# neggles/neurosis

Hardware: AMD Instinct MI355X
Metric: train images/sec (node) SDXL 1024^2 (higher is better)
Workload: dtype bf16

## Files before the change

include/neurosis_hip.h:

```cpp
#ifndef NEUROSIS_HIP_H
#define NEUROSIS_HIP_H

#ifdef __cplusplus
extern "C" {
#endif

const char* nk_last_error(void);
int nk_abi_version(void);

int nk_linear_fwd(const void* x, const void* w, const float* bias, const void* residual, void* y,
                  int M, int N, int K, long ldx, long ldw, long ldr, long ldy, float alpha, void* stream);
int nk_linear_dgrad(const void* dy, const void* w, const void* dx_add, void* dx, int M, int N, int K,
                    long lddy, long ldw, long ldadd, long lddx, void* stream);
long nk_linear_fwd_geglu_ok(int M, int I, int K);
int nk_linear_fwd_geglu(const void* x, const void* w, const float* bias, void* u, void* h, int M, int I, int K, long ldx, long ldw, long ldu,
                        long ldh, void* stream);
int nk_linear_dgrad_geglu(const void* dy, const void* w, const void* u, void* du, int M, int N, int I, long lddy, long ldw, long ldu,
                          long lddu, void* stream);
int nk_linear_fwd_geglu_s(const void* x, const void* w, const float* bias, void* s, void* h, int M, int I, int K, long ldx, long ldw, long lds,
                          long ldh, void* stream);
int nk_linear_dgrad_geglu_s(const void* dy, const void* w, const void* s, void* du, int M, int N, int I, long lddy, long ldw, long lds,
                            long lddu, void* stream);
int nk_linear_wgrad(const void* dy, const void* x, float* dw, int M, int N, int K, long lddy, long ldx,
                    long lddw, int accumulate, void* stream);
// ... 65 lines not shown
int nk_groupnorm_sums(const void* x, float* sums, float* ws, int N, int HW, int C, int G, void* stream);
long nk_groupnorm_sums_ws_floats(int N, int nparts, int G);
int nk_groupnorm_sums_from_parts(const float* part, float* sums, float* ws, int N, int nparts, int G, void* stream);
int nk_groupnorm_apply(const void* x, const float* sums, const float* gamma, const float* beta, void* y, float* mean, float* rstd,
                       int N, int HW, int C, int G, float eps, int silu, void* stream);
int nk_groupnorm_bwd(const void* dy, const void* x, const float* gamma, const float* beta, const float* mean,
                     const float* rstd, const void* dx_add, void* dx, float* dgamma, float* dbeta, float* ws,
                     int N, int HW, int C, int G, int silu, int accumulate, void* stream);
int nk_groupnorm_mod_fwd(const void* x, const float* gamma, const float* beta, const void* mod, void* y, float* mean, float* rstd,
                         float* ws, int N, int HW, int C, int G, float eps, int silu, void* stream);
int nk_groupnorm_mod_apply(const void* x, const float* sums, const float* gamma, const float* beta, const void* mod, void* y, float* mean,
                           float* rstd, int N, int HW, int C, int G, float eps, int silu, void* stream);
int nk_groupnorm_mod_bwd(const void* dy, const void* x, const float* gamma, const float* beta, const void* mod, const float* mean,
                         const float* rstd, const void* dx_add, void* dx, float* dgamma, float* dbeta, void* dmod, float* ws,
                         int N, int HW, int C, int G, int silu, int accumulate, void* stream);

int nk_layernorm_fwd(const void* x, const float* gamma, const float* beta, void* y, float* mean, float* rstd,
                     int M, int C, float eps, void* stream);
long nk_layernorm_ws_floats(int M, int C);
int nk_layernorm_bwd(const void* dy, const void* x, const float* gamma, const float* mean, const float* rstd,
                     const void* dx_add, void* dx, float* dgamma, float* dbeta, float* ws, int M, int C, int accumulate, void* stream);
#define NK_COLPART_MAX 32
typedef struct NkColpartBatch {
  const float* part[NK_COLPART_MAX];
  float* dgamma[NK_COLPART_MAX];
  float* dbeta[NK_COLPART_MAX];
  int nrows[NK_COLPART_MAX];
  int C[NK_COLPART_MAX];
  int accumulate[NK_COLPART_MAX];
  int n;
// ... 142 lines not shown
```

neurosis_amd/csrc/norm.hip:

```cpp
#include "../../include/neurosis_hip.h"
#include "nk_common.h"

#define GN_THREADS 256
#define GN_MAXC 4096

__global__ __launch_bounds__(GN_THREADS) void gn_stats_kernel(const bf16_t* __restrict__ x, float* __restrict__ stats,
                                                              int HW, int C, int G, int rows_per) {
  __shared__ float ps[GN_THREADS * 8], pss[GN_THREADS * 8];
  const int n = blockIdx.y;
  const int cpr = (C >> 3) / gridDim.z;
  const int ch0 = blockIdx.z * cpr;
  const int rows_par = GN_THREADS / cpr;
  const int tid = threadIdx.x;
  const int cpg = C / G;
  const int row_lo = blockIdx.x * rows_per;
  const int row_hi = min(HW, row_lo + rows_per);
  float s[8], ss[8];
#pragma unroll
  for (int e = 0; e < 8; ++e) { s[e] = 0.f; ss[e] = 0.f; }
  const int chunk = tid % cpr, rsub = tid / cpr;
  if (rsub < rows_par) {
    const bf16_t* base = x + ((long)n * HW) * C + (ch0 + chunk) * 8;
    int r = row_lo + rsub;
    for (; r + 3 * rows_par < row_hi; r += 4 * rows_par) {
// ... 21 lines not shown
    }
  }
  __syncthreads();
  float* part = stats + (((long)n * gridDim.x + blockIdx.x) * gridDim.z + blockIdx.z) * 2 * G;
  for (int i = tid; i < 2 * G; i += GN_THREADS) {
    const int g = i >> 1;
    const float* src = (i & 1) ? pss : ps;
    const int c_lo = max(g * cpg, ch0 * 8), c_hi = min((g + 1) * cpg, (ch0 + cpr) * 8);
    float a = 0.f;
    for (int c = c_lo; c < c_hi; ++c)
      for (int r = 0; r < rows_par; ++r) a += src[r * cpr * 8 + (c - ch0 * 8)];
    part[i] = a;
  }
}

__global__ __launch_bounds__(1024) void gn_reduce_partials_kernel(const float* __restrict__ part, float* __restrict__ out,
                                                                 int nparts, int G2) {
  __shared__ float sm[8][128];
  const int n = blockIdx.x;
  const int tx = threadIdx.x & 127, ty = threadIdx.x >> 7;
  float a = 0.f;
  if (tx < G2)
    for (int p = ty; p < nparts; p += 8) a += part[((long)n * nparts + p) * G2 + tx];
  sm[ty][tx] = a;
  __syncthreads();
  if (ty == 0 && tx < G2) {
#pragma unroll
    for (int j = 1; j < 8; ++j) a += sm[j][tx];
    out[(long)n * G2 + tx] = a;
  }
}

__device__ __forceinline__ void gn_modulate(const bf16_t* __restrict__ mod, int n, int c, int C, float& ga, float& be) {
  const float s1 = 1.0f + bf2f(mod[(long)n * 2 * C + c]);
  const float t = bf2f(mod[(long)n * 2 * C + C + c]);
  ga = ga * s1;
  be = be * s1 + t;
}

template <bool MOD>
__global__ __launch_bounds__(GN_THREADS) void gn_apply_kernel(const bf16_t* __restrict__ x, const float* __restrict__ stats,
                                                              const float* __restrict__ gamma, const float* __restrict__ beta,
                                                              const bf16_t* __restrict__ mod,
                                                              bf16_t* __restrict__ y, float* __restrict__ mean_out,
                                                              float* __restrict__ rstd_out, int HW, int C, int G,
                                                              float eps, int silu, int rows_per) {
  extern __shared__ __attribute__((aligned(16))) char smem_raw[];
  float* sc = (float*)smem_raw;
  float* sh = sc + C;
  const int n = blockIdx.y;
  const int tid = threadIdx.x;
  const int cpg = C / G;
  const float inv_cnt = 1.0f / ((float)HW * (float)cpg);
  for (int c = tid; c < C; c += GN_THREADS) {
    int g = c / cpg;
    float m = stats[(long)n * 2 * G + 2 * g] * inv_cnt;
    float var = fmaxf(stats[(long)n * 2 * G + 2 * g + 1] * inv_cnt - m * m, 0.f);
    float rs = rsqrtf(var + eps);
    float ga = gamma[c], be = beta[c];
    if constexpr (MOD) gn_modulate(mod, n, c, C, ga, be);
    float a = rs * ga;
    sc[c] = a;
    sh[c] = be - m * a;
    if (blockIdx.x == 0 && (c % cpg) == 0) { mean_out[n * G + g] = m; rstd_out[n * G + g] = rs; }
  }
  __syncthreads();
  const int cpr = C >> 3;
  const int row_lo = blockIdx.x * rows_per;
  const int row_hi = min(HW, row_lo + rows_per);
  const unsigned total = (unsigned)(row_hi - row_lo) * (unsigned)cpr;
  const bf16_t* xb = x + ((long)n * HW + row_lo) * C;
  bf16_t* yb = y + ((long)n * HW + row_lo) * C;
// ... 180 lines not shown
  if (ty == 0 && c < C) {
#pragma unroll
    for (int j = 1; j < 16; ++j) { a += sa[j][tx]; b += sb[j][tx]; }
    dmod[(long)n * 2 * C + c] = f2bf(gamma[c] * b + beta[c] * a);
    dmod[(long)n * 2 * C + C + c] = f2bf(a);
  }
}

template <bool MOD>
__global__ __launch_bounds__(GN_THREADS) void gn_bwd_apply_kernel(const bf16_t* __restrict__ dy, const bf16_t* __restrict__ x,
                                                                  const float* __restrict__ gamma, const float* __restrict__ beta,
                                                                  const bf16_t* __restrict__ mod,
                                                                  const float* __restrict__ mean, const float* __restrict__ rstd,
                                                                  const float* __restrict__ gsum, const bf16_t* __restrict__ dx_add,
                                                                  bf16_t* __restrict__ dx, int HW, int C, int G, int silu,
                                                                  int rows_per) {
  extern __shared__ __attribute__((aligned(16))) char smem_raw[];
  float* p_a = (float*)smem_raw;
  float* p_b = p_a + C;
  float* p_c = p_b + C;
  float* p_d = p_c + C;
  const int n = blockIdx.y;
  const int tid = threadIdx.x;
  const int cpg = C / G;
  const float inv_cnt = 1.0f / ((float)HW * (float)cpg);
  for (int c = tid; c < C; c += GN_THREADS) {
    const int g = c / cpg;
    const float mu = mean[n * G + g], rs = rstd[n * G + g];
    const float s1 = gsum[(long)n * 2 * G + 2 * g] * inv_cnt, s2 = gsum[(long)n * 2 * G + 2 * g + 1] * inv_cnt;
    float ga = gamma[c], be = beta[c];
    if constexpr (MOD) gn_modulate(mod, n, c, C, ga, be);
    const float a = rs * ga;
    p_a[c] = a;
    p_b[c] = be - mu * a;
    p_c[c] = -rs * rs * s2;
    p_d[c] = -rs * s1 + mu * rs * rs * s2;
  }
  __syncthreads();
  const int cpr = C >> 3;
  const int row_lo = blockIdx.x * rows_per;
  const int row_hi = min(HW, row_lo + rows_per);
  const unsigned total = (unsigned)(row_hi - row_lo) * (unsigned)cpr;
  const long off0 = ((long)n * HW + row_lo) * C;
  auto one = [&](unsigned i, const uint4_t& rx, const uint4_t& rd, const uint4_t& ra) {
// ... 36 lines not shown

static int gn_nz(int C) {
  int cpr = C >> 3, nz = (cpr + GN_THREADS - 1) / GN_THREADS;
  while (cpr % nz) ++nz;
  return nz;
}

static int gn_rows_per(int N, int HW, int* nsplit) {
  int want = (1024 + N - 1) / N;
  int rows_per = (HW + want - 1) / want;
  if (rows_per < 32) rows_per = 32;
  *nsplit = (HW + rows_per - 1) / rows_per;
  return rows_per;
}

extern "C" long nk_groupnorm_ws_floats(int N, int HW, int C, int G) {
  int nsplit;
  gn_rows_per(N, HW, &nsplit);
  long parts = (long)N * nsplit * gn_nz(C) * 2 * G;
  long chan = (long)N * nsplit * 2 * C;
  return parts + chan + (long)N * 2 * G + 64;
}

extern "C" int nk_groupnorm_fwd(const void* x, const float* gamma, const float* beta, void* y, float* mean,
                                float* rstd, float* ws, int N, int HW, int C, int G, float eps, int silu,
                                void* stream_) {
  hipStream_t stream = (hipStream_t)stream_;
  NK_CHECK_ARG(N > 0 && HW > 0 && C > 0 && G > 0 && G <= 64);
  NK_CHECK_ARG((C & 7) == 0 && C % G == 0 && C <= GN_MAXC);
  NK_CHECK_ARG(x && gamma && beta && y && mean && rstd && ws);
  int nsplit;
  int rows_per = gn_rows_per(N, HW, &nsplit);
  const int nz = gn_nz(C);
  float* part = ws;
  float* stats = ws + (long)N * nsplit * nz * 2 * G;
  hipLaunchKernelGGL(gn_stats_kernel, dim3(nsplit, N, nz), dim3(GN_THREADS), 0, stream, (const bf16_t*)x, part, HW, C,
                     G, rows_per);
  if (int e = nk_check_launch("gn_stats_kernel")) return e;
  hipLaunchKernelGGL(gn_reduce_partials_kernel, dim3(N), dim3(1024), 0, stream, part, stats, nsplit * nz, 2 * G);
  if (int e = nk_check_launch("gn_reduce_partials_kernel")) return e;
  hipLaunchKernelGGL(gn_apply_kernel<false>, dim3(nsplit, N), dim3(GN_THREADS), 2 * C * sizeof(float), stream,
                     (const bf16_t*)x, stats, gamma, beta, (const bf16_t*)nullptr, (bf16_t*)y, mean, rstd, HW, C, G, eps, silu, rows_per);
  return nk_check_launch("gn_apply_kernel");
}

__global__ __launch_bounds__(256) void gn_reduce_partials_l1_kernel(const float* __restrict__ part, float* __restrict__ out, int nparts, int G2, int nchunks) {
  __shared__ float sm[4][64];
  const int n = blockIdx.y, chunk = blockIdx.x;
  const int tx = threadIdx.x & 63, ty = threadIdx.x >> 6;
  float a = 0.f;
  if (tx < G2)
    for (int p = chunk + ty * nchunks; p < nparts; p += 4 * nchunks) a += part[((long)n * nparts + p) * G2 + tx];
  sm[ty][tx] = a;
  __syncthreads();
  if (ty == 0 && tx < G2) out[((long)n * nchunks + chunk) * G2 + tx] = (a + sm[1][tx]) + (sm[2][tx] + sm[3][tx]);
}

extern "C" long nk_groupnorm_sums_ws_floats(int N, int nparts, int G) {
// ... 26 lines not shown
  hipLaunchKernelGGL(gn_stats_kernel, dim3(nsplit, N, nz), dim3(GN_THREADS), 0, stream, (const bf16_t*)x, ws, HW, C, G, rows_per);
  if (int e = nk_check_launch("gn_stats_kernel")) return e;
  hipLaunchKernelGGL(gn_reduce_partials_kernel, dim3(N), dim3(1024), 0, stream, ws, sums, nsplit * nz, 2 * G);
  return nk_check_launch("gn_reduce_partials_kernel");
}

extern "C" int nk_groupnorm_apply(const void* x, const float* sums, const float* gamma, const float* beta, void* y, float* mean,
                                  float* rstd, int N, int HW, int C, int G, float eps, int silu, void* stream_) {
  hipStream_t stream = (hipStream_t)stream_;
  NK_CHECK_ARG(N > 0 && HW > 0 && C > 0 && G > 0 && G <= 64);
  NK_CHECK_ARG((C & 7) == 0 && C % G == 0 && C <= GN_MAXC);
  NK_CHECK_ARG(x && sums && gamma && beta && y && mean && rstd);
  int nsplit;
  int rows_per = gn_rows_per(N, HW, &nsplit);
  hipLaunchKernelGGL(gn_apply_kernel<false>, dim3(nsplit, N), dim3(GN_THREADS), 2 * C * sizeof(float), stream, (const bf16_t*)x, sums, gamma, beta,
                     (const bf16_t*)nullptr, (bf16_t*)y, mean, rstd, HW, C, G, eps, silu, rows_per);
  return nk_check_launch("gn_apply_kernel");
}

extern "C" int nk_groupnorm_bwd(const void* dy, const void* x, const float* gamma, const float* beta,
                                const float* mean, const float* rstd, const void* dx_add, void* dx, float* dgamma,
                                float* dbeta, float* ws, int N, int HW, int C, int G, int silu, int accumulate, void* stream_) {
  hipStream_t stream = (hipStream_t)stream_;
  NK_CHECK_ARG(N > 0 && HW > 0 && C > 0 && G > 0 && G <= 64);
  NK_CHECK_ARG((C & 7) == 0 && C % G == 0 && C <= GN_MAXC);
  NK_CHECK_ARG(dy && x && gamma && beta && mean && rstd && dx && dgamma && dbeta && ws);
  int nsplit;
  int rows_per = gn_rows_per(N, HW, &nsplit);
  const int nz = gn_nz(C);
  float* part = ws;
  float* gsum = part + (long)N * nsplit * nz * 2 * G;
  float* chan = gsum + (long)N * 2 * G;
  hipLaunchKernelGGL(gn_bwd_stats_kernel<false>, dim3(nsplit, N, nz), dim3(GN_THREADS), 2 * C * sizeof(float), stream,
                     (const bf16_t*)dy, (const bf16_t*)x, gamma, beta, (const bf16_t*)nullptr, mean, rstd, part, chan, HW, C, G, silu, rows_per);
  if (int e = nk_check_launch("gn_bwd_stats_kernel")) return e;
  hipLaunchKernelGGL(gn_reduce_partials_kernel, dim3(N), dim3(1024), 0, stream, part, gsum, nsplit * nz, 2 * G);
  if (int e = nk_check_launch("gn_reduce_partials_kernel")) return e;
  hipLaunchKernelGGL(colpart_reduce_kernel, dim3((C + 63) / 64), dim3(1024), 0, stream, chan, dgamma, dbeta, N * nsplit, C, accumulate);
  if (int e = nk_check_launch("colpart_reduce_kernel")) return e;
  hipLaunchKernelGGL(gn_bwd_apply_kernel<false>, dim3(nsplit, N), dim3(GN_THREADS), 4 * C * sizeof(float), stream,
                     (const bf16_t*)dy, (const bf16_t*)x, gamma, beta, (const bf16_t*)nullptr, mean, rstd, gsum, (const bf16_t*)dx_add,
                     (bf16_t*)dx, HW, C, G, silu, rows_per);
  return nk_check_launch("gn_bwd_apply_kernel");
}

static int gn_mod_apply_launch(const void* x, const float* sums, const float* gamma, const float* beta, const void* mod, void* y, float* mean,
                               float* rstd, int N, int HW, int C, int G, float eps, int silu, hipStream_t stream) {
  int nsplit;
  int rows_per = gn_rows_per(N, HW, &nsplit);
  hipLaunchKernelGGL(gn_apply_kernel<true>, dim3(nsplit, N), dim3(GN_THREADS), 2 * C * sizeof(float), stream, (const bf16_t*)x, sums, gamma, beta,
                     (const bf16_t*)mod, (bf16_t*)y, mean, rstd, HW, C, G, eps, silu, rows_per);
  return nk_check_launch("gn_apply_kernel<mod>");
}

extern "C" int nk_groupnorm_mod_fwd(const void* x, const float* gamma, const float* beta, const void* mod, void* y, float* mean, float* rstd,
                                    float* ws, int N, int HW, int C, int G, float eps, int silu, void* stream_) {
  hipStream_t stream = (hipStream_t)stream_;
  NK_CHECK_ARG(N > 0 && HW > 0 && C > 0 && G > 0 && G <= 64);
  NK_CHECK_ARG((C & 7) == 0 && C % G == 0 && C <= GN_MAXC);
  NK_CHECK_ARG(x && gamma && beta && mod && y && mean && rstd && ws);
  int nsplit;
  gn_rows_per(N, HW, &nsplit);
  float* stats = ws + (long)N * nsplit * gn_nz(C) * 2 * G;
  if (int e = nk_groupnorm_sums(x, stats, ws, N, HW, C, G, stream_)) return e;
  return gn_mod_apply_launch(x, stats, gamma, beta, mod, y, mean, rstd, N, HW, C, G, eps, silu, stream);
}

extern "C" int nk_groupnorm_mod_apply(const void* x, const float* sums, const float* gamma, const float* beta, const void* mod, void* y,
                                      float* mean, float* rstd, int N, int HW, int C, int G, float eps, int silu, void* stream_) {
  NK_CHECK_ARG(N > 0 && HW > 0 && C > 0 && G > 0 && G <= 64);
  NK_CHECK_ARG((C & 7) == 0 && C % G == 0 && C <= GN_MAXC);
  NK_CHECK_ARG(x && sums && gamma && beta && mod && y && mean && rstd);
  return gn_mod_apply_launch(x, sums, gamma, beta, mod, y, mean, rstd, N, HW, C, G, eps, silu, (hipStream_t)stream_);
}

extern "C" int nk_groupnorm_mod_bwd(const void* dy, const void* x, const float* gamma, const float* beta, const void* mod, const float* mean,
                                    const float* rstd, const void* dx_add, void* dx, float* dgamma, float* dbeta, void* dmod, float* ws,
                                    int N, int HW, int C, int G, int silu, int accumulate, void* stream_) {
  hipStream_t stream = (hipStream_t)stream_;
  NK_CHECK_ARG(N > 0 && HW > 0 && C > 0 && G > 0 && G <= 64);
  NK_CHECK_ARG((C & 7) == 0 && C % G == 0 && C <= GN_MAXC);
  NK_CHECK_ARG(dy && x && gamma && beta && mod && mean && rstd && dx && dgamma && dbeta && dmod && ws);
  int nsplit;
  int rows_per = gn_rows_per(N, HW, &nsplit);
  const int nz = gn_nz(C);
  float* part = ws;
  float* gsum = part + (long)N * nsplit * nz * 2 * G;
  float* chan = gsum + (long)N * 2 * G;
  hipLaunchKernelGGL(gn_bwd_stats_kernel<true>, dim3(nsplit, N, nz), dim3(GN_THREADS), 2 * C * sizeof(float), stream,
                     (const bf16_t*)dy, (const bf16_t*)x, gamma, beta, (const bf16_t*)mod, mean, rstd, part, chan, HW, C, G, silu, rows_per);
  if (int e = nk_check_launch("gn_bwd_stats_kernel<mod>")) return e;
  hipLaunchKernelGGL(gn_reduce_partials_kernel, dim3(N), dim3(1024), 0, stream, part, gsum, nsplit * nz, 2 * G);
  if (int e = nk_check_launch("gn_reduce_partials_kernel")) return e;
  hipLaunchKernelGGL(colpart_reduce_mod_kernel, dim3((C + 63) / 64), dim3(1024), 0, stream, chan, (const bf16_t*)mod, dgamma, dbeta, N * nsplit,
                     nsplit, C, accumulate);
  if (int e = nk_check_launch("colpart_reduce_mod_kernel")) return e;
  hipLaunchKernelGGL(gn_dmod_kernel, dim3((C + 63) / 64, N), dim3(1024), 0, stream, chan, gamma, beta, (bf16_t*)dmod, nsplit, C);
  if (int e = nk_check_launch("gn_dmod_kernel")) return e;
  hipLaunchKernelGGL(gn_bwd_apply_kernel<true>, dim3(nsplit, N), dim3(GN_THREADS), 4 * C * sizeof(float), stream,
                     (const bf16_t*)dy, (const bf16_t*)x, gamma, beta, (const bf16_t*)mod, mean, rstd, gsum, (const bf16_t*)dx_add,
                     (bf16_t*)dx, HW, C, G, silu, rows_per);
  return nk_check_launch("gn_bwd_apply_kernel<mod>");
}

#define LN_MAXCH 4

template <int NCH>
__global__ __launch_bounds__(256) void ln_fwd_kernel(const bf16_t* __restrict__ x, const float* __restrict__ gamma,
                                                     const float* __restrict__ beta, bf16_t* __restrict__ y,
                                                     float* __restrict__ mean, float* __restrict__ rstd, int M, int C,
                                                     float eps) {
  const int lane = threadIdx.x & 63;
  const int wave = (blockIdx.x * blockDim.x + threadIdx.x) >> 6;
  const int nwaves = (gridDim.x * blockDim.x) >> 6;
  const int cpr = C >> 3;
  const float invC = 1.0f / (float)C;
// ... 398 lines not shown
```

neurosis_amd/lib.py:

```python
from __future__ import annotations

import ctypes as C
import os
from pathlib import Path

import torch

CSRC = Path(__file__).resolve().parent / "csrc"
LIB_PATH = CSRC / "libneurosis_hip.so"

vp, i32, i64, f32 = C.c_void_p, C.c_int, C.c_long, C.c_float


class NkConvDesc(C.Structure):
    _fields_ = [(n, i32) for n in ("N", "H", "W", "Cin", "Cout", "KH", "KW", "stride", "pad_t", "pad_l", "Ho", "Wo", "upsample")]


class NkAttnDesc(C.Structure):
    _fields_ = (
        [(n, i32) for n in ("B", "H", "Lq", "Lk", "D")]
        + [(n, i64) for n in ("sq", "sk", "sv", "so", "bq", "bk", "bv", "bo", "sdq", "sdk", "sdv", "sdo", "bdq", "bdk", "bdv", "bdo")]
        + [("scale", f32), ("causal", i32)]
    )

# ... 28 lines not shown
    "nk_conv2d_dgrad_flipped": [cdp, vp, vp, vp, vp],
    "nk_conv2d_wgrad": [cdp, vp, vp, vp, i32, vp],
    "nk_attention_fwd": [adp, vp, vp, vp, vp, vp, vp],
    "nk_attention_bwd": [adp, vp, vp, vp, vp, vp, vp, vp, vp, vp, vp, vp],
    "nk_attention_bwd_causal": [adp, vp, vp, vp, vp, vp, vp, vp, vp, vp, vp],
    "nk_softmax_rows": [vp, i64, i32, vp],
    "nk_softmax_rows_bwd": [vp, vp, i64, i32, f32, vp],
    "nk_groupnorm_fwd": [vp, vp, vp, vp, vp, vp, vp, i32, i32, i32, i32, f32, i32, vp],
    "nk_groupnorm_sums": [vp, vp, vp, i32, i32, i32, i32, vp],
    "nk_groupnorm_sums_from_parts": [vp, vp, vp, i32, i32, i32, vp],
    "nk_groupnorm_apply": [vp, vp, vp, vp, vp, vp, vp, i32, i32, i32, i32, f32, i32, vp],
    "nk_groupnorm_bwd": [vp, vp, vp, vp, vp, vp, vp, vp, vp, vp, vp, i32, i32, i32, i32, i32, i32, vp],
    "nk_groupnorm_mod_fwd": [vp, vp, vp, vp, vp, vp, vp, vp, i32, i32, i32, i32, f32, i32, vp],
    "nk_groupnorm_mod_apply": [vp, vp, vp, vp, vp, vp, vp, vp, i32, i32, i32, i32, f32, i32, vp],
    "nk_groupnorm_mod_bwd": [vp, vp, vp, vp, vp, vp, vp, vp, vp, vp, vp, vp, vp, i32, i32, i32, i32, i32, i32, vp],
    "nk_layernorm_fwd": [vp, vp, vp, vp, vp, vp, i32, i32, f32, vp],
    "nk_layernorm_bwd": [vp, vp, vp, vp, vp, vp, vp, vp, vp, vp, i32, i32, i32, vp],
    "nk_layernorm_bwd_dx": [vp, vp, vp, vp, vp, vp, vp, i32, i32, vp],
    "nk_layernorm_bwd_rows": [vp, vp, vp, vp, vp, vp, vp, vp, i32, i32, vp],
    "nk_colpart_reduce_batch": [C.POINTER(NkColpartBatch), vp],
    "nk_layernorm_bwd_params": [vp, vp, vp, vp, vp, vp, vp, i32, i32, i32, vp],
    "nk_geglu_fwd": [vp, vp, i64, i32, vp],
    "nk_geglu_bwd": [vp, vp, vp, i64, i32, vp],
    "nk_geglu_fwd_s": [vp, vp, vp, i64, i32, vp],
    "nk_geglu_bwd_s": [vp, vp, vp, i64, i32, vp],
    "nk_silu_fwd": [vp, vp, i64, vp],
    "nk_gelu_fwd": [vp, vp, i64, i32, vp],
    "nk_gelu_bwd": [vp, vp, vp, i64, i32, vp],
    "nk_embedding_bwd": [vp, vp, i64, vp, vp, i32, i32, i32, i32, i32, i32, vp],
    "nk_gather_rows_bwd": [vp, i64, vp, vp, i32, i32, i32, vp],
# ... 38 lines not shown
    "nk_debug_raise_health": [vp],
    "nk_debug_stamp": [vp, vp],
    "nk_debug_launch_log": [i32],
    "nk_health_clear": [],
    "nk_health_export": [vp, vp],
    "nk_health_import": [vp, vp],
    "nk_adafactor_init": [vp, vp],
    "nk_adafactor_chunk": [vp, vp],
    "nk_came_chunk": [vp, vp],
    "nk_adamw8bit_step": [vp, vp],
}

SIZE_QUERIES: dict[str, list] = {
    "nk_groupnorm_ws_floats": [i32, i32, i32, i32],
    "nk_groupnorm_sums_ws_floats": [i32, i32, i32],
    "nk_conv2d_stats_tiles": [cdp, i32],
    "nk_conv2d_dgrad_flipped_ok": [cdp],
    "nk_linear_fwd_geglu_ok": [i32, i32, i32],
    "nk_layernorm_ws_floats": [i32, i32],
    "nk_layernorm_part_rows": [i32],
    "nk_colsum_ws_floats": [i64, i32],
    "nk_batchnorm_ws_floats": [i64, i32],
    "nk_lpips_layer_ws_floats": [i32, i32],
    "nk_attention_bwd_ws_floats": [adp],
    "nk_adafactor_tensor_bytes": [],
    "nk_came_tensor_bytes": [],
    "nk_adamw8bit_tensor_bytes": [],
    "nk_gemm_sk_status": [],
    "nk_health_status": [],
    "nk_debug_launch_names": [C.c_char_p, i64],
# ... 58 lines not shown
```

neurosis_amd/ops.py:

```python
from __future__ import annotations

import ctypes as C
import os
import threading
import weakref
from dataclasses import dataclass
from typing import Callable, Optional

import torch
from torch import Tensor

from . import lib
from .lib import NkAttnDesc, NkConvDesc, call, query

BF16 = torch.bfloat16


class EngineState:

    _live = weakref.WeakSet()

    def __init__(self, wgrad_stream=None):
        self.grad_accumulate = False
        self.assume_zeroed = False
# ... 182 lines not shown


def _p(t: Optional[Tensor]):
    return None if t is None else t.data_ptr()


def _stream():
    return torch.cuda.current_stream().cuda_stream


def _check2d(t: Tensor, name: str):
    if t.dim() != 2 or t.stride(1) != 1 or t.dtype != BF16 or not t.is_cuda:
        raise ValueError(f"{name}: expected a 2-D bf16 CUDA tensor with unit inner stride, got {tuple(t.shape)} {t.dtype} {t.stride()} {t.device}")


@dataclass
class Img:

    t: Tensor
    N: int
    H: int
    W: int
    sums: Optional[Tensor] = None

    @property
    def C(self) -> int:
        return self.t.shape[1]

    @staticmethod
    def from_nchw(x: Tensor) -> "Img":
        N, Cc, H, W = x.shape
        if x.dtype == BF16 and x.permute(0, 2, 3, 1).is_contiguous():
            return Img(x.permute(0, 2, 3, 1).reshape(N * H * W, Cc), N, H, W)
        return Img(nchw_to_tokens(x, Cc), N, H, W)

    def to_nchw(self) -> Tensor:
        return self.t.view(self.N, self.H, self.W, self.C).permute(0, 3, 1, 2)

# ... 232 lines not shown
                raise ValueError(f"linear bwd: geglu_u must be [{M}, {2 * K}], got {tuple(geglu_u.shape)}")
            du = torch.empty(M, 2 * K, dtype=BF16, device=dy.device)
            wq = w2d(weight)
            call(entry, dy.data_ptr(), wq.data_ptr(), geglu_u.data_ptr(), du.data_ptr(), M, N, K, dy.stride(0), wq.stride(0),
                 geglu_u.stride(0), du.stride(0), _stream())
            return du
        return gemm_nn(dy, w2d(weight), dx_add)

    return bwd


def _conv_desc(N, H, W, Cin, Cout, KH, KW, stride, pad_t, pad_l, Ho, Wo, upsample) -> NkConvDesc:
    return NkConvDesc(N, H, W, Cin, Cout, KH, KW, stride, pad_t, pad_l, Ho, Wo, int(upsample))


def groupnorm_sums(x: Img, groups: int) -> Tensor:
    if x.sums is not None and x.sums.shape == (x.N, 2 * groups):
        return x.sums
    sums = torch.empty(x.N, 2 * groups, dtype=torch.float32, device=x.t.device)
    ws = _ws(query("nk_groupnorm_ws_floats", x.N, x.H * x.W, x.C, groups), x.t.device)
    call("nk_groupnorm_sums", x.t.data_ptr(), sums.data_ptr(), ws.data_ptr(), x.N, x.H * x.W, x.C, groups, _stream())
    return sums


def conv2d_fwd(x: Img, weight: Tensor, bias: Optional[Tensor], stride: int = 1, padding=1, upsample: bool = False,
               rowvec: Optional[Tensor] = None, residual: Optional[Tensor] = None, need_dx: bool = True,
               asym_pad: bool = False, stats_groups: Optional[int] = None, cin_real: Optional[int] = None):
    Cout, Cin, KH, KW = weight.shape
    if x.C != Cin:
        raise ValueError(f"conv2d: input has {x.C} channels, weight expects {Cin}")
    Hin, Win = (2 * x.H, 2 * x.W) if upsample else (x.H, x.W)
    if asym_pad:
        pad_t = pad_l = 0
        Ho = (Hin + 1 - KH) // stride + 1
        Wo = (Win + 1 - KW) // stride + 1
    else:
        pad_t = pad_l = int(padding)
        Ho = (Hin + 2 * pad_t - KH) // stride + 1
        Wo = (Win + 2 * pad_l - KW) // stride + 1
    d = _conv_desc(x.N, x.H, x.W, Cin, Cout, KH, KW, stride, pad_t, pad_l, Ho, Wo, upsample)
    y = torch.empty(x.N * Ho * Wo, Cout, dtype=BF16, device=x.t.device)
    _check2d(x.t, "x")
    if not x.t.is_contiguous():
        raise ValueError("conv2d: x must be dense channels-last")
    tiles = query("nk_conv2d_stats_tiles", C.byref(d), stats_groups) if stats_groups else 0
    sums_out = None
    if tiles:
        dev = x.t.device
        part = torch.empty(x.N, tiles, 2 * stats_groups, dtype=torch.float32, device=dev)
        call("nk_conv2d_fwd_stats", C.byref(d), x.t.data_ptr(), w2d(weight).data_ptr(), _p(bias), _p(rowvec), _p(residual), y.data_ptr(),
             part.data_ptr(), stats_groups, _stream())
        sums_out = torch.empty(x.N, 2 * stats_groups, dtype=torch.float32, device=dev)
        ws = _ws(query("nk_groupnorm_sums_ws_floats", x.N, tiles, stats_groups), dev)
        call("nk_groupnorm_sums_from_parts", part.data_ptr(), sums_out.data_ptr(), ws.data_ptr(), x.N, tiles, stats_groups, _stream())
    elif (cin_real in (3, 4) and Cin == 8 and KH == 3 and KW == 3 and stride == 1 and pad_t == 1 and not asym_pad and not upsample and rowvec is None
          and residual is None and Cout % 8 == 0):
        call("nk_conv3x3_few_channels_fwd", x.t.data_ptr(), w2d(weight).data_ptr(), _p(bias), y.data_ptr(), x.N, x.H, x.W, Cout, cin_real, _stream())
    else:
        call("nk_conv2d_fwd", C.byref(d), x.t.data_ptr(), w2d(weight).data_ptr(), _p(bias), _p(rowvec), _p(residual), y.data_ptr(), _stream())
    out = Img(y, x.N, Ho, Wo, sums_out)

    def bwd(dy: Tensor):
        _check2d(dy, "dy")
        if not dy.is_contiguous():
            raise ValueError("conv2d bwd: dy must be dense")
        acc = state_of(weight).grad_accumulate

        if weight.requires_grad:
            if bias is not None:
                on_wgrad_stream(lambda: call("nk_conv2d_wgrad_bias", C.byref(d), dy.data_ptr(), x.t.data_ptr(), g2d(weight).data_ptr(), grad_flat(bias).data_ptr(),
                                             wgrad_mode(weight), _stream()), dy, x.t, owner=weight)
            else:
                on_wgrad_stream(lambda: call("nk_conv2d_wgrad", C.byref(d), dy.data_ptr(), x.t.data_ptr(), g2d(weight).data_ptr(), wgrad_mode(weight), _stream()),
                                dy, x.t, owner=weight)
        drow = None
# ... 17 lines not shown
                dxt = dsm
            dx = Img(dxt, x.N, x.H, x.W)
        return dx, drow

    return out, bwd


def groupnorm_fwd(x: Img, weight: Tensor, bias: Tensor, groups: int, eps: float, silu: bool):
    if not x.t.is_contiguous():
        raise ValueError("groupnorm: x must be dense channels-last")
    N, HW, Cc = x.N, x.H * x.W, x.C
    y = torch.empty_like(x.t)
    mean = torch.empty(N, groups, dtype=torch.float32, device=x.t.device)
    rstd = torch.empty_like(mean)
    nws = query("nk_groupnorm_ws_floats", N, HW, Cc, groups)
    if x.sums is not None and x.sums.shape == (N, 2 * groups):
        call("nk_groupnorm_apply", x.t.data_ptr(), x.sums.data_ptr(), weight.data_ptr(), bias.data_ptr(), y.data_ptr(), mean.data_ptr(),
             rstd.data_ptr(), N, HW, Cc, groups, float(eps), int(silu), _stream())
    else:
        ws = _ws(nws, x.t.device)
        call("nk_groupnorm_fwd", x.t.data_ptr(), weight.data_ptr(), bias.data_ptr(), y.data_ptr(), mean.data_ptr(), rstd.data_ptr(),
             ws.data_ptr(), N, HW, Cc, groups, float(eps), int(silu), _stream())

    def bwd(dy: Tensor, dx_add: Optional[Tensor] = None):
        dx = torch.empty_like(x.t)
        ws2 = _ws(nws, dy.device)
        call("nk_groupnorm_bwd", dy.data_ptr(), x.t.data_ptr(), weight.data_ptr(), bias.data_ptr(), mean.data_ptr(), rstd.data_ptr(),
             _p(dx_add), dx.data_ptr(), grad_flat(weight).data_ptr(), grad_flat(bias).data_ptr(), ws2.data_ptr(), N, HW, Cc, groups,
             int(silu), int(state_of(weight).grad_accumulate), _stream())
        return dx

    return Img(y, x.N, x.H, x.W), bwd


def groupnorm_mod_fwd(x: Img, weight: Tensor, bias: Tensor, mod: Tensor, groups: int, eps: float, silu: bool):
    if not x.t.is_contiguous():
        raise ValueError("groupnorm_mod: x must be dense channels-last")
    N, HW, Cc = x.N, x.H * x.W, x.C
    _check2d(mod, "mod")
    if tuple(mod.shape) != (N, 2 * Cc) or not mod.is_contiguous():
        raise ValueError(f"groupnorm_mod: mod must be a dense [{N}, {2 * Cc}] (scale | shift) matrix, got {tuple(mod.shape)}")
    y = torch.empty_like(x.t)
    mean = torch.empty(N, groups, dtype=torch.float32, device=x.t.device)
    rstd = torch.empty_like(mean)
    nws = query("nk_groupnorm_ws_floats", N, HW, Cc, groups)
    if x.sums is not None and x.sums.shape == (N, 2 * groups):
        call("nk_groupnorm_mod_apply", x.t.data_ptr(), x.sums.data_ptr(), weight.data_ptr(), bias.data_ptr(), mod.data_ptr(), y.data_ptr(),
             mean.data_ptr(), rstd.data_ptr(), N, HW, Cc, groups, float(eps), int(silu), _stream())
    else:
        ws = _ws(nws, x.t.device)
        call("nk_groupnorm_mod_fwd", x.t.data_ptr(), weight.data_ptr(), bias.data_ptr(), mod.data_ptr(), y.data_ptr(), mean.data_ptr(),
             rstd.data_ptr(), ws.data_ptr(), N, HW, Cc, groups, float(eps), int(silu), _stream())

    def bwd(dy: Tensor, dx_add: Optional[Tensor] = None):
        dx = torch.empty_like(x.t)
        dmod = torch.empty_like(mod)
        ws2 = _ws(nws, dy.device)
        call("nk_groupnorm_mod_bwd", dy.data_ptr(), x.t.data_ptr(), weight.data_ptr(), bias.data_ptr(), mod.data_ptr(), mean.data_ptr(),
             rstd.data_ptr(), _p(dx_add), dx.data_ptr(), grad_flat(weight).data_ptr(), grad_flat(bias).data_ptr(), dmod.data_ptr(),
             ws2.data_ptr(), N, HW, Cc, groups, int(silu), int(state_of(weight).grad_accumulate), _stream())
        return dx, dmod
# ... 535 lines not shown
```

Measured before the change: 27.26.

## Fold GroupNorm partial-sum reduction into apply kernels to drop separate launches

After: 27.35, median of 6. About the same (+0.3%).

```diff
diff --git a/include/neurosis_hip.h b/include/neurosis_hip.h
--- a/include/neurosis_hip.h
+++ b/include/neurosis_hip.h
@@ -103,6 +103,9 @@
 int nk_groupnorm_mod_bwd(const void* dy, const void* x, const float* gamma, const float* beta, const void* mod, const float* mean,
                          const float* rstd, const void* dx_add, void* dx, float* dgamma, float* dbeta, void* dmod, float* ws,
                          int N, int HW, int C, int G, int silu, int accumulate, void* stream);
+long nk_groupnorm_fold_rows(int nparts, int C);
+int nk_groupnorm_apply_parts(const void* x, const float* part, int nparts, const float* gamma, const float* beta, const void* mod, void* y,
+                             float* mean, float* rstd, int N, int HW, int C, int G, float eps, int silu, void* stream);
 
 int nk_layernorm_fwd(const void* x, const float* gamma, const float* beta, void* y, float* mean, float* rstd,
                      int M, int C, float eps, void* stream);
diff --git a/neurosis_amd/csrc/norm.hip b/neurosis_amd/csrc/norm.hip
--- a/neurosis_amd/csrc/norm.hip
+++ b/neurosis_amd/csrc/norm.hip
@@ -1,5 +1,6 @@
 #include "../../include/neurosis_hip.h"
 #include "nk_common.h"
+#include <stdlib.h>
 
 #define GN_THREADS 256
 #define GN_MAXC 4096
@@ -59,21 +60,56 @@
   }
 }
 
+template <int NT, int CW>
+__device__ __forceinline__ void gn_sum_partials(const float* __restrict__ part_n, int nparts, int G2, float (*sm)[128], int tid) {
+  constexpr int TSTEP = NT / CW, NCH = TSTEP >= 8 ? 1 : 8 / TSTEP;
+  const int tx = tid % CW, ty0 = tid / CW;
+  if (ty0 < 8) {
+    float a[NCH];
+#pragma unroll
+    for (int k = 0; k < NCH; ++k) a[k] = 0.f;
+    if (tx < G2) {
+      int p0 = 0;
+#pragma unroll 4
+      for (; p0 + 8 <= nparts; p0 += 8) {
+#pragma unroll
+        for (int k = 0; k < NCH; ++k) a[k] += part_n[(long)(p0 + ty0 + k * TSTEP) * G2 + tx];
+      }
+#pragma unroll
+      for (int k = 0; k < NCH; ++k)
+        if (p0 + ty0 + k * TSTEP < nparts) a[k] += part_n[(long)(p0 + ty0 + k * TSTEP) * G2 + tx];
+    }
+#pragma unroll
+    for (int k = 0; k < NCH; ++k) sm[ty0 + k * TSTEP][tx] = a[k];
+  }
+  __syncthreads();
+}
+__device__ __forceinline__ float gn_partials_total(float (*sm)[128], int col) {
+  float a = sm[0][col];
+#pragma unroll
+  for (int j = 1; j < 8; ++j) a += sm[j][col];
+  return a;
+}
+
+#define GN_FOLD_ROWS 256
+#define GN_FOLD_LDS (9 * 128 * (int)sizeof(float))
+static bool gn_fold_rows(long rows, int coef_floats) {
+  const char* e = getenv("NK_GN_FOLD");
+  return !(e && e[0] == '0' && !e[1]) && rows >= 1 && rows <= GN_FOLD_ROWS && coef_floats * (long)sizeof(float) + GN_FOLD_LDS <= 65536;
+}
+__device__ __forceinline__ void gn_fold_prologue(const float* __restrict__ part_n, int nparts, int G2, float (*sm)[128], float* tot, int tid) {
+  if (G2 <= 64) gn_sum_partials<GN_THREADS, 64>(part_n, nparts, G2, sm, tid);
+  else gn_sum_partials<GN_THREADS, 128>(part_n, nparts, G2, sm, tid);
+  if (tid < G2) tot[tid] = gn_partials_total(sm, tid);
+  __syncthreads();
+}
+
 __global__ __launch_bounds__(1024) void gn_reduce_partials_kernel(const float* __restrict__ part, float* __restrict__ out,
                                                                  int nparts, int G2) {
   __shared__ float sm[8][128];
   const int n = blockIdx.x;
-  const int tx = threadIdx.x & 127, ty = threadIdx.x >> 7;
-  float a = 0.f;
-  if (tx < G2)
-    for (int p = ty; p < nparts; p += 8) a += part[((long)n * nparts + p) * G2 + tx];
-  sm[ty][tx] = a;
-  __syncthreads();
-  if (ty == 0 && tx < G2) {
-#pragma unroll
-    for (int j = 1; j < 8; ++j) a += sm[j][tx];
-    out[(long)n * G2 + tx] = a;
-  }
+  gn_sum_partials<1024, 128>(part + (long)n * nparts * G2, nparts, G2, sm, threadIdx.x);
+  if (threadIdx.x < G2) out[(long)n * G2 + threadIdx.x] = gn_partials_total(sm, threadIdx.x);
 }
 
 __device__ __forceinline__ void gn_modulate(const bf16_t* __restrict__ mod, int n, int c, int C, float& ga, float& be) {
@@ -89,18 +125,25 @@
                                                               const bf16_t* __restrict__ mod,
                                                               bf16_t* __restrict__ y, float* __restrict__ mean_out,
                                                               float* __restrict__ rstd_out, int HW, int C, int G,
-                                                              float eps, int silu, int rows_per) {
+                                                              float eps, int silu, int rows_per, int nparts) {
   extern __shared__ __attribute__((aligned(16))) char smem_raw[];
   float* sc = (float*)smem_raw;
   float* sh = sc + C;
+  float (*fold_sm)[128] = (float (*)[128])(sh + C);
+  float* fold_tot = sh + C + 8 * 128;
   const int n = blockIdx.y;
   const int tid = threadIdx.x;
   const int cpg = C / G;
   const float inv_cnt = 1.0f / ((float)HW * (float)cpg);
+  const float* st = stats + (long)n * 2 * G;
+  if (nparts > 0) {
+    gn_fold_prologue(stats + (long)n * nparts * 2 * G, nparts, 2 * G, fold_sm, fold_tot, tid);
+    st = fold_tot;
+  }
   for (int c = tid; c < C; c += GN_THREADS) {
     int g = c / cpg;
-    float m = stats[(long)n * 2 * G + 2 * g] * inv_cnt;
-    float var = fmaxf(stats[(long)n * 2 * G + 2 * g + 1] * inv_cnt - m * m, 0.f);
+    float m = st[2 * g] * inv_cnt;
+    float var = fmaxf(st[2 * g + 1] * inv_cnt - m * m, 0.f);
     float rs = rsqrtf(var + eps);
     float ga = gamma[c], be = beta[c];
     if constexpr (MOD) gn_modulate(mod, n, c, C, ga, be);
@@ -311,20 +354,27 @@
                                                                   const float* __restrict__ mean, const float* __restrict__ rstd,
                                                                   const float* __restrict__ gsum, const bf16_t* __restrict__ dx_add,
                                                                   bf16_t* __restrict__ dx, int HW, int C, int G, int silu,
-                                                                  int rows_per) {
+                                                                  int rows_per, int nparts) {
   extern __shared__ __attribute__((aligned(16))) char smem_raw[];
   float* p_a = (float*)smem_raw;
   float* p_b = p_a + C;
   float* p_c = p_b + C;
   float* p_d = p_c + C;
+  float (*fold_sm)[128] = (float (*)[128])(p_d + C);
+  float* fold_tot = p_d + C + 8 * 128;
   const int n = blockIdx.y;
   const int tid = threadIdx.x;
   const int cpg = C / G;
   const float inv_cnt = 1.0f / ((float)HW * (float)cpg);
+  const float* gs = gsum + (long)n * 2 * G;
+  if (nparts > 0) {
+    gn_fold_prologue(gsum + (long)n * nparts * 2 * G, nparts, 2 * G, fold_sm, fold_tot, tid);
+    gs = fold_tot;
+  }
   for (int c = tid; c < C; c += GN_THREADS) {
     const int g = c / cpg;
     const float mu = mean[n * G + g], rs = rstd[n * G + g];
-    const float s1 = gsum[(long)n * 2 * G + 2 * g] * inv_cnt, s2 = gsum[(long)n * 2 * G + 2 * g + 1] * inv_cnt;
+    const float s1 = gs[2 * g] * inv_cnt, s2 = gs[2 * g + 1] * inv_cnt;
     float ga = gamma[c], be = beta[c];
     if constexpr (MOD) gn_modulate(mod, n, c, C, ga, be);
     const float a = rs * ga;
@@ -391,6 +441,28 @@
   return rows_per;
 }
 
+static int gn_apply_launch(const void* x, const float* part, int nparts, float* sums, const float* gamma, const float* beta, const void* mod,
+                           void* y, float* mean, float* rstd, int N, int HW, int C, int G, float eps, int silu, hipStream_t stream) {
+  int nsplit;
+  const int rows_per = gn_rows_per(N, HW, &nsplit);
+  const bool fold = gn_fold_rows(nparts, 2 * C);
+  if (!fold) {
+    NK_CHECK_ARG(sums != nullptr);
+    hipLaunchKernelGGL(gn_reduce_partials_kernel, dim3(N), dim3(1024), 0, stream, part, sums, nparts, 2 * G);
+    if (int e = nk_check_launch("gn_reduce_partials_kernel")) return e;
+  }
+  const float* st = fold ? part : sums;
+  const size_t lds = 2 * C * sizeof(float) + (fold ? GN_FOLD_LDS : 0);
+  if (mod) {
+    hipLaunchKernelGGL(gn_apply_kernel<true>, dim3(nsplit, N), dim3(GN_THREADS), lds, stream, (const bf16_t*)x, st, gamma, beta,
+                       (const bf16_t*)mod, (bf16_t*)y, mean, rstd, HW, C, G, eps, silu, rows_per, fold ? nparts : 0);
+    return nk_check_launch("gn_apply_kernel<mod>");
+  }
+  hipLaunchKernelGGL(gn_apply_kernel<false>, dim3(nsplit, N), dim3(GN_THREADS), lds, stream, (const bf16_t*)x, st, gamma, beta,
+                     (const bf16_t*)nullptr, (bf16_t*)y, mean, rstd, HW, C, G, eps, silu, rows_per, fold ? nparts : 0);
+  return nk_check_launch("gn_apply_kernel");
+}
+
 extern "C" long nk_groupnorm_ws_floats(int N, int HW, int C, int G) {
   int nsplit;
   gn_rows_per(N, HW, &nsplit);
@@ -414,11 +486,7 @@
   hipLaunchKernelGGL(gn_stats_kernel, dim3(nsplit, N, nz), dim3(GN_THREADS), 0, stream, (const bf16_t*)x, part, HW, C,
                      G, rows_per);
   if (int e = nk_check_launch("gn_stats_kernel")) return e;
-  hipLaunchKernelGGL(gn_reduce_partials_kernel, dim3(N), dim3(1024), 0, stream, part, stats, nsplit * nz, 2 * G);
-  if (int e = nk_check_launch("gn_reduce_partials_kernel")) return e;
-  hipLaunchKernelGGL(gn_apply_kernel<false>, dim3(nsplit, N), dim3(GN_THREADS), 2 * C * sizeof(float), stream,
-                     (const bf16_t*)x, stats, gamma, beta, (const bf16_t*)nullptr, (bf16_t*)y, mean, rstd, HW, C, G, eps, silu, rows_per);
-  return nk_check_launch("gn_apply_kernel");
+  return gn_apply_launch(x, part, nsplit * nz, stats, gamma, beta, nullptr, y, mean, rstd, N, HW, C, G, eps, silu, stream);
 }
 
 __global__ __launch_bounds__(256) void gn_reduce_partials_l1_kernel(const float* __restrict__ part, float* __restrict__ out, int nparts, int G2, int nchunks) {
@@ -475,7 +543,7 @@
   int nsplit;
   int rows_per = gn_rows_per(N, HW, &nsplit);
   hipLaunchKernelGGL(gn_apply_kernel<false>, dim3(nsplit, N), dim3(GN_THREADS), 2 * C * sizeof(float), stream, (const bf16_t*)x, sums, gamma, beta,
-                     (const bf16_t*)nullptr, (bf16_t*)y, mean, rstd, HW, C, G, eps, silu, rows_per);
+                     (const bf16_t*)nullptr, (bf16_t*)y, mean, rstd, HW, C, G, eps, silu, rows_per, 0);
   return nk_check_launch("gn_apply_kernel");
 }
 
@@ -495,13 +563,16 @@
   hipLaunchKernelGGL(gn_bwd_stats_kernel<false>, dim3(nsplit, N, nz), dim3(GN_THREADS), 2 * C * sizeof(float), stream,
                      (const bf16_t*)dy, (const bf16_t*)x, gamma, beta, (const bf16_t*)nullptr, mean, rstd, part, chan, HW, C, G, silu, rows_per);
   if (int e = nk_check_launch("gn_bwd_stats_kernel")) return e;
-  hipLaunchKernelGGL(gn_reduce_partials_kernel, dim3(N), dim3(1024), 0, stream, part, gsum, nsplit * nz, 2 * G);
-  if (int e = nk_check_launch("gn_reduce_partials_kernel")) return e;
+  const bool fold = gn_fold_rows(nsplit * nz, 4 * C);
+  if (!fold) {
+    hipLaunchKernelGGL(gn_reduce_partials_kernel, dim3(N), dim3(1024), 0, stream, part, gsum, nsplit * nz, 2 * G);
+    if (int e = nk_check_launch("gn_reduce_partials_kernel")) return e;
+  }
   hipLaunchKernelGGL(colpart_reduce_kernel, dim3((C + 63) / 64), dim3(1024), 0, stream, chan, dgamma, dbeta, N * nsplit, C, accumulate);
   if (int e = nk_check_launch("colpart_reduce_kernel")) return e;
-  hipLaunchKernelGGL(gn_bwd_apply_kernel<false>, dim3(nsplit, N), dim3(GN_THREADS), 4 * C * sizeof(float), stream,
-                     (const bf16_t*)dy, (const bf16_t*)x, gamma, beta, (const bf16_t*)nullptr, mean, rstd, gsum, (const bf16_t*)dx_add,
-                     (bf16_t*)dx, HW, C, G, silu, rows_per);
+  hipLaunchKernelGGL(gn_bwd_apply_kernel<false>, dim3(nsplit, N), dim3(GN_THREADS), 4 * C * sizeof(float) + (fold ? GN_FOLD_LDS : 0), stream,
+                     (const bf16_t*)dy, (const bf16_t*)x, gamma, beta, (const bf16_t*)nullptr, mean, rstd, fold ? part : gsum, (const bf16_t*)dx_add,
+                     (bf16_t*)dx, HW, C, G, silu, rows_per, fold ? nsplit * nz : 0);
   return nk_check_launch("gn_bwd_apply_kernel");
 }
 
@@ -510,7 +581,7 @@
   int nsplit;
   int rows_per = gn_rows_per(N, HW, &nsplit);
   hipLaunchKernelGGL(gn_apply_kernel<true>, dim3(nsplit, N), dim3(GN_THREADS), 2 * C * sizeof(float), stream, (const bf16_t*)x, sums, gamma, beta,
-                     (const bf16_t*)mod, (bf16_t*)y, mean, rstd, HW, C, G, eps, silu, rows_per);
+                     (const bf16_t*)mod, (bf16_t*)y, mean, rstd, HW, C, G, eps, silu, rows_per, 0);
   return nk_check_launch("gn_apply_kernel<mod>");
 }
 
@@ -522,9 +593,11 @@
   NK_CHECK_ARG(x && gamma && beta && mod && y && mean && rstd && ws);
   int nsplit;
   gn_rows_per(N, HW, &nsplit);
-  float* stats = ws + (long)N * nsplit * gn_nz(C) * 2 * G;
-  if (int e = nk_groupnorm_sums(x, stats, ws, N, HW, C, G, stream_)) return e;
-  return gn_mod_apply_launch(x, stats, gamma, beta, mod, y, mean, rstd, N, HW, C, G, eps, silu, stream);
+  const int rows_per = gn_rows_per(N, HW, &nsplit), nz = gn_nz(C);
+  float* stats = ws + (long)N * nsplit * nz * 2 * G;
+  hipLaunchKernelGGL(gn_stats_kernel, dim3(nsplit, N, nz), dim3(GN_THREADS), 0, stream, (const bf16_t*)x, ws, HW, C, G, rows_per);
+  if (int e = nk_check_launch("gn_stats_kernel")) return e;
+  return gn_apply_launch(x, ws, nsplit * nz, stats, gamma, beta, mod, y, mean, rstd, N, HW, C, G, eps, silu, stream);
 }
 
 extern "C" int nk_groupnorm_mod_apply(const void* x, const float* sums, const float* gamma, const float* beta, const void* mod, void* y,
@@ -533,6 +606,16 @@
   NK_CHECK_ARG((C & 7) == 0 && C % G == 0 && C <= GN_MAXC);
   NK_CHECK_ARG(x && sums && gamma && beta && mod && y && mean && rstd);
   return gn_mod_apply_launch(x, sums, gamma, beta, mod, y, mean, rstd, N, HW, C, G, eps, silu, (hipStream_t)stream_);
+}
+
+extern "C" long nk_groupnorm_fold_rows(int nparts, int C) { return gn_fold_rows(nparts, 2 * C) ? 1 : 0; }
+extern "C" int nk_groupnorm_apply_parts(const void* x, const float* part, int nparts, const float* gamma, const float* beta, const void* mod,
+                                        void* y, float* mean, float* rstd, int N, int HW, int C, int G, float eps, int silu, void* stream_) {
+  NK_CHECK_ARG(N > 0 && HW > 0 && C > 0 && G > 0 && G <= 64);
+  NK_CHECK_ARG((C & 7) == 0 && C % G == 0 && C <= GN_MAXC);
+  NK_CHECK_ARG(x && part && gamma && beta && y && mean && rstd);
+  NK_CHECK_ARG(gn_fold_rows(nparts, 2 * C));
+  return gn_apply_launch(x, part, nparts, nullptr, gamma, beta, mod, y, mean, rstd, N, HW, C, G, eps, silu, (hipStream_t)stream_);
 }
 
 extern "C" int nk_groupnorm_mod_bwd(const void* dy, const void* x, const float* gamma, const float* beta, const void* mod, const float* mean,
@@ -551,16 +634,19 @@
   hipLaunchKernelGGL(gn_bwd_stats_kernel<true>, dim3(nsplit, N, nz), dim3(GN_THREADS), 2 * C * sizeof(float), stream,
                      (const bf16_t*)dy, (const bf16_t*)x, gamma, beta, (const bf16_t*)mod, mean, rstd, part, chan, HW, C, G, silu, rows_per);
   if (int e = nk_check_launch("gn_bwd_stats_kernel<mod>")) return e;
-  hipLaunchKernelGGL(gn_reduce_partials_kernel, dim3(N), dim3(1024), 0, stream, part, gsum, nsplit * nz, 2 * G);
-  if (int e = nk_check_launch("gn_reduce_partials_kernel")) return e;
+  const bool fold = gn_fold_rows(nsplit * nz, 4 * C);
+  if (!fold) {
+    hipLaunchKernelGGL(gn_reduce_partials_kernel, dim3(N), dim3(1024), 0, stream, part, gsum, nsplit * nz, 2 * G);
+    if (int e = nk_check_launch("gn_reduce_partials_kernel")) return e;
+  }
   hipLaunchKernelGGL(colpart_reduce_mod_kernel, dim3((C + 63) / 64), dim3(1024), 0, stream, chan, (const bf16_t*)mod, dgamma, dbeta, N * nsplit,
                      nsplit, C, accumulate);
   if (int e = nk_check_launch("colpart_reduce_mod_kernel")) return e;
   hipLaunchKernelGGL(gn_dmod_kernel, dim3((C + 63) / 64, N), dim3(1024), 0, stream, chan, gamma, beta, (bf16_t*)dmod, nsplit, C);
   if (int e = nk_check_launch("gn_dmod_kernel")) return e;
-  hipLaunchKernelGGL(gn_bwd_apply_kernel<true>, dim3(nsplit, N), dim3(GN_THREADS), 4 * C * sizeof(float), stream,
-                     (const bf16_t*)dy, (const bf16_t*)x, gamma, beta, (const bf16_t*)mod, mean, rstd, gsum, (const bf16_t*)dx_add,
-                     (bf16_t*)dx, HW, C, G, silu, rows_per);
+  hipLaunchKernelGGL(gn_bwd_apply_kernel<true>, dim3(nsplit, N), dim3(GN_THREADS), 4 * C * sizeof(float) + (fold ? GN_FOLD_LDS : 0), stream,
+                     (const bf16_t*)dy, (const bf16_t*)x, gamma, beta, (const bf16_t*)mod, mean, rstd, fold ? part : gsum, (const bf16_t*)dx_add,
+                     (bf16_t*)dx, HW, C, G, silu, rows_per, fold ? nsplit * nz : 0);
   return nk_check_launch("gn_bwd_apply_kernel<mod>");
 }
 
diff --git a/neurosis_amd/lib.py b/neurosis_amd/lib.py
--- a/neurosis_amd/lib.py
+++ b/neurosis_amd/lib.py
@@ -66,6 +66,7 @@
     "nk_groupnorm_mod_fwd": [vp, vp, vp, vp, vp, vp, vp, vp, i32, i32, i32, i32, f32, i32, vp],
     "nk_groupnorm_mod_apply": [vp, vp, vp, vp, vp, vp, vp, vp, i32, i32, i32, i32, f32, i32, vp],
     "nk_groupnorm_mod_bwd": [vp, vp, vp, vp, vp, vp, vp, vp, vp, vp, vp, vp, vp, i32, i32, i32, i32, i32, i32, vp],
+    "nk_groupnorm_apply_parts": [vp, vp, i32, vp, vp, vp, vp, vp, vp, i32, i32, i32, i32, f32, i32, vp],
     "nk_layernorm_fwd": [vp, vp, vp, vp, vp, vp, i32, i32, f32, vp],
     "nk_layernorm_bwd": [vp, vp, vp, vp, vp, vp, vp, vp, vp, vp, i32, i32, i32, vp],
     "nk_layernorm_bwd_dx": [vp, vp, vp, vp, vp, vp, vp, i32, i32, vp],
@@ -134,6 +135,7 @@
 SIZE_QUERIES: dict[str, list] = {
     "nk_groupnorm_ws_floats": [i32, i32, i32, i32],
     "nk_groupnorm_sums_ws_floats": [i32, i32, i32],
+    "nk_groupnorm_fold_rows": [i32, i32],
     "nk_conv2d_stats_tiles": [cdp, i32],
     "nk_conv2d_dgrad_flipped_ok": [cdp],
     "nk_linear_fwd_geglu_ok": [i32, i32, i32],
diff --git a/neurosis_amd/ops.py b/neurosis_amd/ops.py
--- a/neurosis_amd/ops.py
+++ b/neurosis_amd/ops.py
@@ -4,7 +4,6 @@
 import os
 import threading
 import weakref
-from dataclasses import dataclass
 from typing import Callable, Optional
 
 import torch
@@ -220,14 +219,25 @@
         raise ValueError(f"{name}: expected a 2-D bf16 CUDA tensor with unit inner stride, got {tuple(t.shape)} {t.dtype} {t.stride()} {t.device}")
 
 
-@dataclass
 class Img:
 
-    t: Tensor
-    N: int
-    H: int
-    W: int
-    sums: Optional[Tensor] = None
+    def __init__(self, t: Tensor, N: int, H: int, W: int, sums: Optional[Tensor] = None, parts: Optional[Tensor] = None):
+        self.t, self.N, self.H, self.W = t, N, H, W
+        self._sums = sums
+        self.parts = parts
+
+    def __repr__(self) -> str:
+        return f"Img(t={self.t!r}, N={self.N}, H={self.H}, W={self.W}, sums={self._sums!r}, parts={self.parts!r})"
+
+    @property
+    def sums(self) -> Optional[Tensor]:
+        if self._sums is None and self.parts is not None:
+            self._sums = _sums_from_parts(self.parts)
+        return self._sums
+
+    @sums.setter
+    def sums(self, value: Optional[Tensor]) -> None:
+        self._sums, self.parts = value, None
 
     @property
     def C(self) -> int:
@@ -490,6 +500,21 @@
     return NkConvDesc(N, H, W, Cin, Cout, KH, KW, stride, pad_t, pad_l, Ho, Wo, int(upsample))
 
 
+def _sums_from_parts(part: Tensor) -> Tensor:
+    n, tiles, g2 = part.shape
+    sums = torch.empty(n, g2, dtype=torch.float32, device=part.device)
+    ws = _ws(query("nk_groupnorm_sums_ws_floats", n, tiles, g2 // 2), part.device)
+    call("nk_groupnorm_sums_from_parts", part.data_ptr(), sums.data_ptr(), ws.data_ptr(), n, tiles, g2 // 2, _stream())
+    return sums
+
+
+def _foldable_parts(x: Img, groups: int) -> Optional[Tensor]:
+    p = x.parts
+    if p is None or x._sums is not None or p.shape[0] != x.N or p.shape[2] != 2 * groups:
+        return None
+    return p if query("nk_groupnorm_fold_rows", p.shape[1], x.C) else None
+
+
 def groupnorm_sums(x: Img, groups: int) -> Tensor:
     if x.sums is not None and x.sums.shape == (x.N, 2 * groups):
         return x.sums
@@ -520,21 +545,19 @@
     if not x.t.is_contiguous():
         raise ValueError("conv2d: x must be dense channels-last")
     tiles = query("nk_conv2d_stats_tiles", C.byref(d), stats_groups) if stats_groups else 0
-    sums_out = None
+    sums_out = part = None
     if tiles:
-        dev = x.t.device
-        part = torch.empty(x.N, tiles, 2 * stats_groups, dtype=torch.float32, device=dev)
+        part = torch.empty(x.N, tiles, 2 * stats_groups, dtype=torch.float32, device=x.t.device)
         call("nk_conv2d_fwd_stats", C.byref(d), x.t.data_ptr(), w2d(weight).data_ptr(), _p(bias), _p(rowvec), _p(residual), y.data_ptr(),
              part.data_ptr(), stats_groups, _stream())
-        sums_out = torch.empty(x.N, 2 * stats_groups, dtype=torch.float32, device=dev)
-        ws = _ws(query("nk_groupnorm_sums_ws_floats", x.N, tiles, stats_groups), dev)
-        call("nk_groupnorm_sums_from_parts", part.data_ptr(), sums_out.data_ptr(), ws.data_ptr(), x.N, tiles, stats_groups, _stream())
+        if not query("nk_groupnorm_fold_rows", tiles, Cout):
+            sums_out, part = _sums_from_parts(part), None
     elif (cin_real in (3, 4) and Cin == 8 and KH == 3 and KW == 3 and stride == 1 and pad_t == 1 and not asym_pad and not upsample and rowvec is None
           and residual is None and Cout % 8 == 0):
         call("nk_conv3x3_few_channels_fwd", x.t.data_ptr(), w2d(weight).data_ptr(), _p(bias), y.data_ptr(), x.N, x.H, x.W, Cout, cin_real, _stream())
     else:
         call("nk_conv2d_fwd", C.byref(d), x.t.data_ptr(), w2d(weight).data_ptr(), _p(bias), _p(rowvec), _p(residual), y.data_ptr(), _stream())
-    out = Img(y, x.N, Ho, Wo, sums_out)
+    out = Img(y, x.N, Ho, Wo, sums_out, part)
 
     def bwd(dy: Tensor):
         _check2d(dy, "dy")
@@ -582,7 +605,11 @@
     mean = torch.empty(N, groups, dtype=torch.float32, device=x.t.device)
     rstd = torch.empty_like(mean)
     nws = query("nk_groupnorm_ws_floats", N, HW, Cc, groups)
-    if x.sums is not None and x.sums.shape == (N, 2 * groups):
+    part = _foldable_parts(x, groups)
+    if part is not None:
+        call("nk_groupnorm_apply_parts", x.t.data_ptr(), part.data_ptr(), part.shape[1], weight.data_ptr(), bias.data_ptr(), None, y.data_ptr(),
+             mean.data_ptr(), rstd.data_ptr(), N, HW, Cc, groups, float(eps), int(silu), _stream())
+    elif x.sums is not None and x.sums.shape == (N, 2 * groups):
         call("nk_groupnorm_apply", x.t.data_ptr(), x.sums.data_ptr(), weight.data_ptr(), bias.data_ptr(), y.data_ptr(), mean.data_ptr(),
              rstd.data_ptr(), N, HW, Cc, groups, float(eps), int(silu), _stream())
     else:
@@ -612,7 +639,11 @@
     mean = torch.empty(N, groups, dtype=torch.float32, device=x.t.device)
     rstd = torch.empty_like(mean)
     nws = query("nk_groupnorm_ws_floats", N, HW, Cc, groups)
-    if x.sums is not None and x.sums.shape == (N, 2 * groups):
+    part = _foldable_parts(x, groups)
+    if part is not None:
+        call("nk_groupnorm_apply_parts", x.t.data_ptr(), part.data_ptr(), part.shape[1], weight.data_ptr(), bias.data_ptr(), mod.data_ptr(),
+             y.data_ptr(), mean.data_ptr(), rstd.data_ptr(), N, HW, Cc, groups, float(eps), int(silu), _stream())
+    elif x.sums is not None and x.sums.shape == (N, 2 * groups):
         call("nk_groupnorm_mod_apply", x.t.data_ptr(), x.sums.data_ptr(), weight.data_ptr(), bias.data_ptr(), mod.data_ptr(), y.data_ptr(),
              mean.data_ptr(), rstd.data_ptr(), N, HW, Cc, groups, float(eps), int(silu), _stream())
     else:
```
